# eigenkernel/eigenkernel

Measured on AMD Instinct MI355X. Metric: eigenpairs/s (full spectrum) + achieved fp64 TFLOP/s vs roofline, N=16384 GEP, higher is better.
Workload: dtype f64

## Files before the change

eigenkernel_amd/csrc/ek_api.hip:

```cpp
#include "ek_api_internal.h"

#include <cfloat>

namespace ek {
namespace api {

Context g_ctx;
std::mutex g_mu;

int ensure_init() {
  if (g_ctx.ready) return 0;
  int ndev = 0;
  EK_HIP_CHECK(hipGetDeviceCount(&ndev));
  if (ndev <= 0) {
    fprintf(stderr, "[ek_hip] no HIP device visible: this library has no CPU fallback\n");
    return -1000 - (int)hipErrorNoDevice;
  }
  EK_HIP_CHECK(hipSetDevice(g_ctx.device));
  EK_HIP_CHECK(hipStreamCreateWithFlags(&g_ctx.stream, hipStreamNonBlocking));
  {
    int lo = 0, hi = 0;
    (void)hipDeviceGetStreamPriorityRange(&lo, &hi);
    EK_HIP_CHECK(hipStreamCreateWithPriority(&g_ctx.stream2, hipStreamNonBlocking, hi));
  }
  EK_HIP_CHECK(hipMalloc((void **)&g_ctx.d_info, 64 * sizeof(int)));
  EK_HIP_CHECK(hipMalloc((void **)&g_ctx.d_status, 64));
  EK_HIP_CHECK(hipMalloc((void **)&g_ctx.d_stats, 64));
  EK_HIP_CHECK(hipMemset(g_ctx.d_stats, 0, 64));
  g_ctx.ready = true;
  return 0;
}

namespace { void *g_uimg = nullptr; size_t g_uimg_bytes = 0; }
int user_images(size_t bytes, void **p) {
  if (bytes > g_uimg_bytes) {
    if (g_uimg) EK_HIP_CHECK(hipFree(g_uimg));
    g_uimg = nullptr; g_uimg_bytes = 0;
    EK_HIP_CHECK(hipMalloc(&g_uimg, bytes));
// ... 853 lines not shown
```

eigenkernel_amd/csrc/ek_api_internal.h:

```cpp
#pragma once
#include "../../include/ek_hip.h"
#include "../../include/ek_hip_debug.h"
#include "ek_common.h"
#include "ek_switch.h"

#include <rccl/rccl.h>

#include <chrono>
#include <cstdlib>
#include <cstring>
#include <mutex>
#include <vector>

namespace ek {
namespace batched {
struct Desc {
  double *A, *B, *w, *Z;
  int n, lda, ldb, ldz, index, pad;
};
static_assert(sizeof(Desc) == 56, "the table's entry");
struct WDesc {
  double vl, vu;
  int il, iu, zcap, wcols;
  long long lu;
};
static_assert(sizeof(WDesc) == 40, "the window table's entry");
}

namespace api {

struct Context {
  bool ready = false;
  int device = 0;
  hipStream_t stream = nullptr;
  hipStream_t stream2 = nullptr;
  void *ws = nullptr;
  void *ws_alloc = nullptr;
  size_t ws_bytes = 0;
  int *d_info = nullptr;
  double *d_status = nullptr;
  double *d_stats = nullptr;
  double stats[8] = {0, 0, 0, 0, 0, 0, 0, 0};
};
extern Context g_ctx;
extern std::mutex g_mu;

int ensure_init();
int workspace(size_t bytes, void **p);

struct Arena {
// ... 52 lines not shown
int d2h_matrix(int m, int n, const double *d, int ldd, double *h, int ldh, hipStream_t s);
int fetch_info(int *info);
void poison_foreign_strips(hipStream_t s, int n, double *A, int lda, int P, int rank);
void count_mismatch(hipStream_t s, int m, int n, const double *X, int ldx, const double *Y, int ldy, int lower,
                    unsigned long long *count);

struct Comm {
  bool on = false;
  bool host = false;
  ncclComm_t comm = nullptr;
  int nranks = 0, rank = 0;
  int err = 0;
};
extern Comm g_comm;
constexpr int kPotrfRlMin = 1024;
extern int g_two_stage_min;
int two_stage_min();
int dist_min_ranks();
void comm_teardown();
SytrdExchange team_exchange(int nteam, int n = 0);
void team_sendrecv(hipStream_t s, int npeers, const int *peers, double *const *send, const size_t *send_counts,
                   double *const *recv, const size_t *recv_counts);
int comm_any(int local);
int comm_agree(int local_rc);
const char *comm_error_string();

void gather_band_strips(hipStream_t s, int n, int nmem, int rank0, double *const *ABs, const SytrdExchange &x);

inline int hip_rc(hipError_t e) { return e == hipSuccess ? 0 : -1000 - (int)e; }
#define EK_TRY(call) do { const int rc_ = (call); if (rc_) return rc_; } while (0)
// ... 57 lines not shown
```

eigenkernel_amd/csrc/ek_chol.hip:

```cpp
#include "ek_common.h"
#include "ek_block64.h"

#include <cstdlib>
#include <vector>

namespace ek {
namespace {

constexpr int NB = kDiagNB;
constexpr size_t kDiagLds = 2 * b64::IMG * sizeof(double);

__global__ __launch_bounds__(256) void potrf_diag_kernel(int nb, double *B, int ldb, double *inv, int *info,
                                                         int info_base) {
  using namespace b64;
  extern __shared__ double smem[];
  double *sP = smem, *sQ = smem + IMG;
  __shared__ double s_scr[kScratch];
  const int t = threadIdx.x, lane = t & 63, wave = t >> 6, l15 = lane & 15, l4 = lane >> 4;
  auto upper = [&](int gr, int gc) -> double {
    if (gc < nb) return B[(size_t)gc + (size_t)gr * ldb];
    return (gr == gc) ? 1.0 : 0.0;
  };
  auto fail_exit = [&](int j) {
    if (t == 0) atomicCAS(info, 0, info_base + j + 1);
// ... 198 lines not shown
  static bool attr_set = false;
  if (attr_set) return;
  (void)hipFuncSetAttribute((const void *)potrf_diag_kernel, hipFuncAttributeMaxDynamicSharedMemorySize, kDiagLds);
  (void)hipFuncSetAttribute((const void *)trtri_diag_kernel,
                            hipFuncAttributeMaxDynamicSharedMemorySize, (NB * NB + NB) * sizeof(double));
  attr_set = true;
}

void potrf_lower(hipStream_t s, int n, double *B, int ldb, double *invdiag, int *d_info,
                 double *work) {
  set_attrs();
  if (n <= 0) return;
  potrf_rec(s, n, B, ldb, 0, invdiag, d_info, work);
}

void trtri256_blocks(hipStream_t s, int n, const double *L, int ldl, const double *invdiag, double *inv256, double *scratch) {
  const int nb2 = n / (2 * NB);
  if (nb2 <= 0) return;
  GemmDesc g{};
  g.M = NB; g.N = NB; g.K = NB; g.transA = false; g.transB = false; g.alpha = 1.0; g.beta = 0.0; g.batch = nb2; g.lower_only = false;
  g.A = L + NB; g.lda = ldl; g.strideA = (long long)2 * NB * ((long long)ldl + 1);
  g.B = invdiag; g.ldb = NB; g.strideB = (long long)2 * NB * NB;
  g.C = scratch; g.ldc = NB; g.strideC = (long long)NB * NB;
  gemm(s, g);
  g.alpha = -1.0;
  g.A = invdiag + (size_t)NB * NB; g.lda = NB; g.strideA = (long long)2 * NB * NB;
  g.B = scratch; g.ldb = NB; g.strideB = (long long)NB * NB;
  g.C = inv256 + NB; g.ldc = 2 * NB; g.strideC = (long long)4 * NB * NB;
  gemm(s, g);
  hipLaunchKernelGGL(inv256_assemble_kernel, dim3(nb2), dim3(256), 0, s, invdiag, inv256);
}
void trsm_register_inv256(const double *invdiag, const double *inv256, int n) {
  g_inv256.base128 = inv256 ? invdiag : nullptr; g_inv256.inv256 = inv256; g_inv256.nblk256 = inv256 ? n / (2 * NB) : 0;
// ... 124 lines not shown
  const int before = g_sygst_direct;
  g_sygst_direct = order <= 0 ? kSygstDirect : (order < 2 * NB ? 2 * NB : order);
  return before;
}
void sygst_scratch_need(int n, size_t need[2]) {
  if (n <= sygst_direct()) return;
  const size_t n1 = (size_t)split_t(n), n2 = (size_t)n - n1;
  const size_t t1 = n1 * n1 + n1 * n2, t2 = (n1 > n2 ? n1 : n2) * (size_t)n;
  if (t1 > need[0]) need[0] = t1;
  if (t2 > need[1]) need[1] = t2;
  sygst_scratch_need((int)n1, need);
  sygst_scratch_need((int)n2, need);
}

static void sygst_rec(hipStream_t s, int n, double *A, int lda, const double *L, int ldl,
                      const double *invdiag, double *work, double *scratch) {
  if (n <= 0) return;
  if (n <= sygst_direct()) {
    symmetrize_lower(s, n, A, lda);
    trsm_lln(s, n, n, L, ldl, invdiag, A, lda, work);
    trsm_rlt_lower(s, n, L, ldl, invdiag, A, lda, work);
    return;
  }
  const int n1 = split_t(n), n2 = n - n1;
  double *A21 = A + n1, *A22 = A + (size_t)n1 + (size_t)n1 * lda;
  const double *L21 = L + n1, *L22 = L + (size_t)n1 + (size_t)n1 * ldl;
  const double *inv2 = invdiag + (size_t)(n1 / NB) * NB * NB;
  sygst_rec(s, n1, A, lda, L, ldl, invdiag, work, scratch);
  trsm_rlt(s, n2, n1, L, ldl, invdiag, A21, lda, work);
  double *C11 = scratch, *M = scratch + (size_t)n1 * n1;
  hipLaunchKernelGGL(full_from_lower_kernel, grid_mn(n1, n1), dim3(256), 0, s, n1, A, lda, C11, n1);
  gemm(s, false, false, n2, n1, n1, 1.0, L21, ldl, C11, n1, 0.0, M, n2);
  hipLaunchKernelGGL(axpy_matrix_kernel, grid_mn(n2, n1), dim3(256), 0, s, n2, n1, -0.5, M, n2, A21, lda);
  if (n2 <= n1) {
    double *P = C11;
    gemm(s, false, true, n2, n2, n1, 1.0, A21, lda, L21, ldl, 0.0, P, n2);
    hipLaunchKernelGGL(syr2k_fold_kernel, dim3(ceil_div(n2, 32), ceil_div(n2, 32)), dim3(256), 0, s, n2, P, n2, A22, lda);
  } else {
    gemm(s, false, true, n2, n2, n1, -1.0, A21, lda, L21, ldl, 1.0, A22, lda, true);
    gemm(s, false, true, n2, n2, n1, -1.0, L21, ldl, A21, lda, 1.0, A22, lda, true);
  }
  hipLaunchKernelGGL(axpy_matrix_kernel, grid_mn(n2, n1), dim3(256), 0, s, n2, n1, -0.5, M, n2, A21, lda);
  trsm_lln(s, n2, n1, L22, ldl, inv2, A21, lda, work);
  sygst_rec(s, n2, A22, lda, L22, ldl, inv2, work, scratch);
}

void sygst_lower(hipStream_t s, int n, double *A, int lda, const double *L, int ldl,
                 const double *invdiag, double *work, double *scratch) {
  if (n <= 0) return;
  sygst_rec(s, n, A, lda, L, ldl, invdiag, work, scratch);
}


__global__ __launch_bounds__(256) void trmm_diag_kernel(int n, int ldd, const double *__restrict__ L, int ldl,
                                                        double *__restrict__ diag) {
  const int b = blockIdx.x, off = b * ldd;
  const int nb = n - off < ldd ? n - off : ldd;
  double *D = diag + (size_t)b * ldd * ldd;
  const int per = ldd * ldd / gridDim.y;
  for (int idx = blockIdx.y * per + threadIdx.x; idx < (blockIdx.y + 1) * per; idx += 256) {
    const int i = idx % ldd, j = idx / ldd;
    D[idx] = (i >= j && i < nb) ? L[(size_t)(off + i) + (size_t)(off + j) * ldl] : 0.0;
  }
}
int trmm_block_ld(int n) { return n > kDiagNB ? 2 * NB : NB; }
// ... 288 lines not shown
      if (e0) { g_pprof.mark(s); g_pprof.kind.push_back(1); }
      if (has_next) issue_strip(s, k + 1, cur ^ 1);
      waited = true;
    }
  }
  for (int m = 0; m < nmem; ++m)
    hipLaunchKernelGGL(info_to_double_kernel, dim3(ceil_div(NRB, 256)), dim3(256), 0, s, NRB, infos[m], infod[m]);
  x.allreduce(s, nmem, infod, (size_t)NRB, x.user);
  for (int m = 0; m < nmem; ++m)
    hipLaunchKernelGGL(first_info_kernel, dim3(1), dim3(64), 0, s, NRB, infod[m], mem[m].d_info);
}

size_t potrf_rl_work_bytes(int n, int ld) { return PotrfDistLayout(n, ld, 1).total; }

void potrf_lower_rl(hipStream_t s, hipStream_t s2, int n, double *B, int ldb, double *invdiag, int *d_info,
                    void *work) {
  set_attrs();
  if (n <= 0) return;
  const PotrfDistLayout Ly(n, ldb, 1);
  const int NRB = Ly.NRB;
  char *w = (char *)work;
  double *ppan = (double *)(w + Ly.off_pbuf);
  int *infos = (int *)(w + Ly.off_infos);
  double *infod = (double *)(w + Ly.off_infod);
  long long *offs = (long long *)(w + Ly.off_offs);
  int *dims = (int *)(w + Ly.off_dims);
  static hipEvent_t evU[2], evP[2], evFork;
  static bool ev_ready = false;
  if (!ev_ready) {
    for (int i = 0; i < 2; ++i) {
      (void)hipEventCreateWithFlags(&evU[i], hipEventDisableTiming);
      (void)hipEventCreateWithFlags(&evP[i], hipEventDisableTiming);
    }
    (void)hipEventCreateWithFlags(&evFork, hipEventDisableTiming);
    ev_ready = true;
  }
  (void)hipMemsetAsync(infos, 0, (size_t)NRB * sizeof(int), s);
  hipLaunchKernelGGL(potrf_table_kernel, dim3(NRB), dim3(round_up(Ly.maxb, 64)), 0, s, n, ldb, 1, 0, NRB, Ly.maxb,
                     offs, dims);
  auto factor_panel = [&](hipStream_t st, int k) {
    const int off = k * NB, nbk = (n - off < NB) ? n - off : NB, mrows = n - off - nbk;
    double *Bd = B + (size_t)off + (size_t)off * ldb;
    double *inv = invdiag + (size_t)k * NB * NB;
    hipLaunchKernelGGL(potrf_diag_kernel, dim3(1), dim3(256), kDiagLds, st, nbk, Bd,
                       ldb, inv, infos + k, off);
    if (mrows > 0) {
      gemm(st, false, true, mrows, nbk, nbk, 1.0, Bd + nbk, ldb, inv, NB, 0.0, ppan, mrows);
      copy_matrix(st, mrows, nbk, ppan, mrows, Bd + nbk, ldb);
    }
// ... 5 lines not shown
    for (int k = k0; k < k1; ++k) {
      factor_panel(st, k);
      const int cnt = k1 - 1 - k;
      if (cnt > 0) {
        const int nbk = (n - k * NB < NB) ? n - k * NB : NB;
        GemmDesc g{};
        g.N = NB; g.K = nbk; g.transA = false; g.transB = true; g.alpha = -1.0; g.beta = 1.0;
        g.A = B; g.lda = ldb; g.B = B; g.ldb = ldb; g.C = B; g.ldc = ldb; g.lower_only = true;
        g.even_offs = true;
        g.M = n - (k + 1) * NB; g.batch = cnt;
        g.d_offs = offs + (size_t)k * Ly.maxb * 3; g.d_dims = dims + (size_t)k * Ly.maxb * 3;
        gemm(st, g);
      }
    }
  };
  (void)hipEventRecord(evFork, s);
  (void)hipStreamWaitEvent(s2, evFork, 0);
  factor_outer(s2, 0);
  (void)hipEventRecord(evP[0], s2);
  for (int o = 0; o + 1 < NOB; ++o) {
    const int c0 = o * ob * NB, c1 = (o + 1) * ob * NB, kw = c1 - c0;
    const int m2 = n - c1;
    const int wnext = (m2 < ob * NB) ? m2 : ob * NB;
    (void)hipStreamWaitEvent(s, evP[o & 1], 0);
    const double *P = B + (size_t)c1 + (size_t)c0 * ldb;
    double *C = B + (size_t)c1 + (size_t)c1 * ldb;
    gemm(s, false, true, m2, wnext, kw, -1.0, P, ldb, P, ldb, 1.0, C, ldb, true);
    (void)hipEventRecord(evU[(o + 1) & 1], s);
    if (m2 > wnext)
      gemm(s, false, true, m2 - wnext, m2 - wnext, kw, -1.0, P + wnext, ldb, P + wnext, ldb, 1.0,
           C + (size_t)wnext + (size_t)wnext * ldb, ldb, true);
    (void)hipStreamWaitEvent(s2, evU[(o + 1) & 1], 0);
    factor_outer(s2, o + 1);
    (void)hipEventRecord(evP[(o + 1) & 1], s2);
  }
  (void)hipStreamWaitEvent(s, evP[(NOB - 1) & 1], 0);
  hipLaunchKernelGGL(info_to_double_kernel, dim3(ceil_div(NRB, 256)), dim3(256), 0, s, NRB, infos, infod);
  hipLaunchKernelGGL(first_info_kernel, dim3(1), dim3(64), 0, s, NRB, infod, d_info);
}

size_t sygst_dist_scratch_doubles(int n, int ld, int nranks) {
  const int NRB = ceil_div(n > 0 ? n : 1, NB);
  return (size_t)ld * NB * ceil_div(NRB, nranks > 0 ? nranks : 1);
}

void sygst_lower_dist(hipStream_t s, int n, int nmem, const SygstMember *mem, const SytrdExchange &x) {
  if (n <= 0 || nmem <= 0 || nmem > kMaxTeam) return;
  const int P = x.nranks;
  const int NRB = ceil_div(n, NB);
  const int wblk = ceil_div(NRB, P) * NB;
  size_t offs[kMaxTeam], counts[kMaxTeam];
  for (int r = 0; r < P; ++r) {
    long long c0 = (long long)r * wblk, c1 = c0 + wblk;
// ... 34 lines not shown
```

eigenkernel_amd/csrc/ek_common.h:

```cpp
#pragma once
#include <hip/hip_runtime.h>
#include <cstddef>
#include <cstdint>
#include <cstdio>

#define EK_HIP_CHECK(expr)                                                              \
  do {                                                                                  \
    hipError_t _e = (expr);                                                             \
    if (_e != hipSuccess) {                                                             \
      fprintf(stderr, "[ek_hip] %s failed at %s:%d: %s\n", #expr, __FILE__, __LINE__,   \
              hipGetErrorString(_e));                                                   \
      return -1000 - (int)_e;                                                           \
    }                                                                                   \
  } while (0)

namespace ek {

constexpr int kWave = 64;

inline int ceil_div(int a, int b) { return (a + b - 1) / b; }
inline int round_up(int a, int b) { return ceil_div(a, b) * b; }

struct GemmDesc {
  int M, N, K;
// ... 59 lines not shown
constexpr int kDiagNB = 128;
void potrf_lower(hipStream_t s, int n, double *B, int ldb, double *invdiag, int *d_info,
                 double *work );
void trtri_diag_blocks(hipStream_t s, int n, const double *L, int ldl, double *invdiag);
void trsm_rlt(hipStream_t s, int m, int n, const double *L, int ldl, const double *invdiag,
              double *X, int ldx, double *work);
void trsm_lln(hipStream_t s, int n, int m, const double *L, int ldl, const double *invdiag,
              double *X, int ldx, double *work);
void trsm_llt(hipStream_t s, int n, int m, const double *L, int ldl, const double *invdiag,
              double *X, int ldx, double *work);
inline size_t sygst_scratch_doubles(int n) {
  const size_t h = (size_t)(n / 2 + 128);
  const size_t a = 2 * h * h, b = 2 * 128 * 128;
  return a > b ? a : b;
}
void trtri256_blocks(hipStream_t s, int n, const double *L, int ldl, const double *invdiag, double *inv256, double *scratch);
void trsm_register_inv256(const double *invdiag, const double *inv256, int n);
void sygst_lower(hipStream_t s, int n, double *A, int lda, const double *L, int ldl,
                 const double *invdiag, double *work, double *scratch);
int sygst_set_direct(int order);
void sygst_scratch_need(int n, size_t need[2]);
int trmm_block_ld(int n);
size_t trmm_diag_doubles(int n);
void trmm_diag_blocks(hipStream_t s, int n, const double *L, int ldl, double *diag);
void trmm_rln(hipStream_t s, int m, int n, const double *L, int ldl, const double *diag, int ldd,
              double *X, int ldx, double *work);
void trmm_llt(hipStream_t s, int n, int m, const double *L, int ldl, const double *diag, int ldd,
              double *X, int ldx, double *work);
void trmm_lln(hipStream_t s, int n, int m, const double *L, int ldl, const double *diag, int ldd,
              double *X, int ldx, double *work);
void sygst2_lower(hipStream_t s, int n, double *A, int lda, const double *L, int ldl, const double *diag,
                  double *work, double *scratch);
struct SygstMember {
  double *A; int lda; const double *L; int ldl; const double *invdiag;
  double *work;
  double *scratch;
  int rank;
};
size_t potrf_rl_work_bytes(int n, int ld);
void potrf_lower_rl(hipStream_t s, hipStream_t s2, int n, double *B, int ldb, double *invdiag, int *d_info,
                    void *work);
struct SytrdExchange;
struct PotrfMember { double *B; int ldb; double *invdiag; int *d_info; void *work; int rank; };
size_t potrf_dist_work_bytes(int n, int ld, int nranks);
void potrf_lower_dist(hipStream_t s, hipStream_t s2, int n, int nmem, const PotrfMember *mem, const SytrdExchange &x);
void potrf_dist_set_lookahead(int on);
void potrf_dist_profile(bool on);
void potrf_dist_profile_collect(double *seconds, int P);
size_t sygst_dist_scratch_doubles(int n, int ld, int nranks);
void sygst_lower_dist(hipStream_t s, int n, int nmem, const SygstMember *mem, const SytrdExchange &x);

struct SytrdWork;
size_t sytrd_work_bytes(int n);
void sytrd_lower(hipStream_t s, int n, double *A, int lda, double *d, double *e, double *tau,
                 double *V, int ldv, void *work);

// ... 105 lines not shown
```

eigenkernel_amd/csrc/ek_debug.hip:

```cpp
#include "ek_api_internal.h"

using namespace ek;
using namespace ek::api;

extern "C" {

int ek_hip_potrf_team(int n, double *B_loc, const int desc_B[9], int nteam, long long *mismatch) {
  if (n < 0) return -1;
  if (!B_loc && n > 0) return -2;
  int rc = check_desc(desc_B, 3, n, n); if (rc) return rc;
  if (nteam < 0 || nteam > kMaxTeam) return -4;
  rc = ensure_init(); if (rc) return rc;
  if (mismatch) *mismatch = 0;
  if (n == 0) return 0;
  std::lock_guard<std::mutex> lk(g_mu);
  if (nteam == 0 && !g_comm.on) return -4;
  hipStream_t s = g_ctx.stream;
  const int ld = pad_ld(n), nblk = ceil_div(n, kDiagNB);
  const int nmem = nteam > 0 ? nteam : 1, P = nteam > 0 ? nteam : g_comm.nranks;
  const size_t wb = potrf_dist_work_bytes(n, ld, P);
  const size_t per = al((size_t)ld * ld * 8) + al((size_t)nblk * kDiagNB * kDiagNB * 8) + al(wb) + 256;
  void *ws;
  rc = workspace(per * nmem + 256, &ws);
  if (rc) return rc;
// ... 206 lines not shown
  return sy2sb_on_host_arrays(n, A, lda, V, ldv, tau, 0, flag);
}

int ek_hip_debug_sy2sb_stage(int n, double *A, int lda, double *V, int ldv, double *tau, int poison, int *flag) {
  if (n < 1) return -1;
  if (!A) return -2;
  if (lda < n) return -3;
  if (!V) return -4;
  if (ldv < n) return -5;
  if (!tau) return -6;
  if (!flag) return -8;
  return sy2sb_on_host_arrays(n, A, lda, V, ldv, tau, poison, flag);
}

int ek_hip_debug_set_sy2sb_flow(int pair_min, int lookahead_min) { sy2sb_set_flow(pair_min, lookahead_min); return 0; }

__global__ void band_to_matrix_kernel(int n, const double *__restrict__ AB, double *__restrict__ A, int lda) {
  const int c = blockIdx.x;
  for (int d = threadIdx.x; d <= kBandW; d += blockDim.x)
    if (c + d < n) A[(size_t)(c + d) + (size_t)c * lda] = AB[(size_t)d + (size_t)c * kBandLd];
}

int ek_hip_debug_sy2sb_team(int n, double *A, int lda, double *V, int ldv, double *tau, int nteam, int *flag,
                            long long *mismatch) {
  if (n < 1 || !A || !V || !tau || lda < n || ldv < n) return -1;
  if (nteam < 0 || nteam > kMaxTeam) return -7;
  int rc = ensure_init(); if (rc) return rc;
  std::lock_guard<std::mutex> lk(g_mu);
  if (nteam == 0 && !g_comm.on) return -7;
  hipStream_t s = g_ctx.stream;
// ... 705 lines not shown
```

eigenkernel_amd/csrc/ek_solve.hip:

```cpp
#include "ek_api_internal.h"

namespace ek {
namespace api {

void gather_band_strips(hipStream_t s, int n, int nmem, int rank0, double *const *ABs, const SytrdExchange &x) {
  const int NRB = ceil_div(n, 128), P = x.nranks;
  if (P <= 1) return;
  for (int q = 0; q * P < NRB; ++q) {
    size_t offs[kMaxTeam], counts[kMaxTeam];
    for (int r = 0; r < P; ++r) {
      const int S = q * P + r;
      const int cols = (S < NRB) ? ((n - S * 128 < 128) ? n - S * 128 : 128) : 0;
      offs[r] = (S < NRB) ? (size_t)S * 128 * kBandLd : 0; counts[r] = (size_t)cols * kBandLd;
    }
    x.allgatherv(s, nmem, rank0, ABs, offs, counts, P, x.user);
  }
}

}
}

using namespace ek;
using namespace ek::api;

namespace {

struct StageTimer {
  hipEvent_t ev[EK_HIP_N_STAGES + 1];
  int made = 0;
  int init() {
    for (auto &e : ev) { EK_HIP_CHECK(hipEventCreate(&e)); ++made; }
    return 0;
// ... 20 lines not shown
  p.two_stage = ts_min > 0 && n >= ts_min && n >= 3;
  p.mat = al((size_t)p.ld * p.ld * 8);
  p.compact_dc = stedc_compact(n, nc_loc);
  p.zcols = p.compact_dc ? round_up(nc_loc > 0 ? nc_loc : 1, 128) : p.ld;
  p.zmat = al((size_t)p.ld * p.zcols * 8);
  p.wb_sytrd = (p.two_stage) ? 0 : (dist ? sytrd_dist_work_bytes(n, nranks_dist) : sytrd_work_bytes(n));
  p.wb_stedc = stedc_work_bytes(n, nc_loc);
  p.wb_ormtr = ormtr_work_bytes(n, nc_loc, n_vec);
  p.trsm_work = al((size_t)256 * p.ld * 8);
  p.inv256 = (problem == 1) ? al((size_t)(n / 256 > 0 ? n / 256 : 1) * 256 * 256 * 8) : 0;
  p.sygst_dbl = (problem == 1) ? sygst_scratch_doubles(n) : 0;
  if (problem == 1 && dist) {
    const size_t dd = sygst_dist_scratch_doubles(n, p.ld, nranks_dist);
    if (dd > p.sygst_dbl) p.sygst_dbl = dd;
  }
  p.potrf_rl = problem == 1 && n >= kPotrfRlMin;
  p.potrf_wb = (problem == 1 && dist) ? al(potrf_dist_work_bytes(n, p.ld, nranks_dist)) : 0;
  if (p.potrf_rl && al(potrf_rl_work_bytes(n, p.ld)) > p.potrf_wb) p.potrf_wb = al(potrf_rl_work_bytes(n, p.ld));
  p.wb_sy2sb = p.two_stage ? al(dist ? sy2sb_dist_work_bytes(n, nranks_dist) : sy2sb_work_bytes(n)) : 0;
  p.wb_sb2st = p.two_stage ? al(sb2st_work_bytes(n, false)) : 0;
  p.wb_rec = p.two_stage ? al(sb2st_record_bytes(n)) : 0;
  p.wb_q1prep = p.two_stage ? al(ormtr_prep_bytes(n)) : 0;
  p.x0 = p.mat;
  const size_t phase_a = al(p.sygst_dbl * 8) + p.potrf_wb + al(p.wb_sytrd) + 512;
  p.x1 = phase_a;
  if (values_only) {
    p.zcols = 0; p.zmat = 0; p.wb_stedc = 0; p.wb_ormtr = 0; p.wb_rec = 0; p.wb_q1prep = 0;
    if (al(stebz_work_bytes(n)) > p.x1) p.x1 = al(stebz_work_bytes(n));
    if (p.x1 < 4096) p.x1 = 4096;
  }
  if (al(p.wb_stedc) > p.x1) p.x1 = al(p.wb_stedc);
// ... 20 lines not shown
  int run();
  int rc = 0;
  hipStream_t s = g_ctx.stream;
  int nc_out = 0, nr_loc = 0, nc_loc = 0;
  bool dist = false, split_rows = false, values_only = false, value_window = false;
  PathPlan pl{};
  int ld = 0;
  bool two_stage = false, aliasA = false, aliasB = false, aliasZ = false;
  double *wB = nullptr, *wV = nullptr, *wZ = nullptr, *x0 = nullptr, *dInv = nullptr, *twork = nullptr, *dd = nullptr,
         *de = nullptr, *dt = nullptr, *dwv = nullptr, *dt1 = nullptr, *inv256 = nullptr;
  char *x1 = nullptr, *work_sy2sb = nullptr, *work_sb2st = nullptr, *q1prep = nullptr;
  double *wA = nullptr, *wV2 = nullptr;
  double *sscr = nullptr; char *pwork = nullptr; void *sytrd_work = nullptr;
  char *work = nullptr; double *q2rec = nullptr;
  Inv256Guard inv256_guard;
  StageTimer tm;
  bool timing = false;
  int evi = 0;
  void mark() { if (timing) (void)hipEventRecord(tm.ev[evi++], s); }
  double sigma = 1.0;
  bool band_input = false;
  bool two_stage_done = false, window_too_small = false;
  double rescued_panels = 0.0;
  int zslab = 0;
  int stage_in_A(), stage_in_B(), reduce(), tridiagonalise(), chase_with_repeat(), count_window(), values_tail(),
      divide_and_conquer(), stage_out(), finish(bool full), slab_width(int c0) const;
  void cholesky(), a_out(), back_transform(), recover(), z_out(int c0, int nc), exchange_rows();
};

Path::Path(const PathCall &call) : PathCall(call) {
// ... 34 lines not shown
  dd = a.get<double>(ld); de = a.get<double>(ld); dt = a.get<double>(ld); dwv = a.get<double>(ld);
  dt1 = a.get<double>(ld);
  work_sy2sb = two_stage ? a.get<char>(pl.wb_sy2sb) : nullptr;
  work_sb2st = two_stage ? a.get<char>(pl.wb_sb2st) : nullptr;
  q1prep = (two_stage && !values_only) ? a.get<char>(pl.wb_q1prep) : nullptr;
  inv256 = pl.inv256 ? (double *)a.get<char>(pl.inv256) : nullptr;
  wA = aliasA ? dA : x0;
  wV2 = x0;
  sscr = (problem == 1) ? (double *)x1 : nullptr;
  pwork = pl.potrf_wb ? x1 + al(pl.sygst_dbl * 8) : nullptr;
  work = x1;
  q2rec = (double *)x1;
  char *sytrd_arena = x1 + al(pl.sygst_dbl * 8) + pl.potrf_wb + 256;
  sytrd_work = two_stage ? nullptr : choose_sytrd_scratch(n, ld, x0, sytrd_arena, dd, pl.wb_sytrd);
  timing = stage_seconds && n_stages > 0;
}

int Path::run() {
  if (rc) return rc;
  if (timing) EK_TRY(tm.init());
  EK_HIP_CHECK(hipMemsetAsync(g_ctx.d_info, 0, 4 * sizeof(int), s));
  mark();
  EK_HIP_CHECK(hipMemsetAsync(wV, 0, (size_t)ld * ld * 8, s));
  EK_HIP_CHECK(hipMemsetAsync(dd, 0, 4 * al((size_t)ld * 8), s));
  if (!pipe) EK_TRY(stage_in_A());
  EK_TRY(stage_in_B());
  mark();
  cholesky();
  mark();
  if (pipe) {
    EK_TRY(stage_in_A());
    if (problem == 1) {
      if (!aliasB) copy_matrix(s, n, n, wB, ld, dB, ldb);
      pipe_out(pipe, s, 'B', dB, ldb, n, 0, n);
    }
  }
  EK_TRY(reduce());
  mark();
  EK_TRY(tridiagonalise());
  mark();
  EK_TRY(count_window());
  if (values_only || (win && (win->m == 0 || window_too_small))) return values_tail();
  EK_TRY(divide_and_conquer());
  mark();
  back_transform();
  mark();
  recover();
  mark();
  EK_TRY(stage_out());
  mark();
  return finish(true);
}
// ... 22 lines not shown
  for (int q = 0; q < 256; ++q) { if (part[q] > anrm) anrm = part[q]; if (!(part[256 + q] <= offband)) offband = part[256 + q]; }
  band_input = switch_int(kSwBandInput) != 0 && problem == 0 && !dist && offband == 0.0;
  if (!(anrm <= 1.7e308)) return -4;
  const double rmin = 1e-90, rmax = 1e90;
  if (anrm > 0.0 && anrm < rmin) sigma = rmin / anrm;
  else if (anrm > rmax) sigma = rmax / anrm;
  if (sigma != 1.0) scale_lower(s, n, sigma, wA, ld);
  return 0;
}

void Path::cholesky() {
  if (problem == 1) {
    if (dist && g_comm.nranks >= dist_min_ranks()) {
      const PotrfMember me{wB, ld, dInv, g_ctx.d_info, pwork, g_comm.rank};
      potrf_lower_dist(s, g_ctx.stream2, n, 1, &me, team_exchange(0));
    } else if (pl.potrf_rl) {
      potrf_lower_rl(s, g_ctx.stream2, n, wB, ld, dInv, g_ctx.d_info, pwork);
    } else {
      potrf_lower(s, n, wB, ld, dInv, g_ctx.d_info, twork);
    }
  }
  if (problem == 1 && n >= 256 && (itype == 1 || (itype == 2 && !values_only))) {
    trtri256_blocks(s, n, wB, ld, dInv, inv256, twork);
    trsm_register_inv256(dInv, inv256, n);
  }
}

int Path::reduce() {
  if (problem != 1) return 0;
  if (dist && g_comm.nranks >= dist_min_ranks()) {
    const SygstMember me{wA, ld, wB, ld, dInv, twork, sscr, g_comm.rank};
    sygst_lower_dist(s, n, 1, &me, team_exchange(0));
  } else if (itype == 1) {
    sygst_lower(s, n, wA, ld, wB, ld, dInv, twork, sscr);
  } else {
    trmm_diag_blocks(s, n, wB, ld, wV);
    sygst2_lower(s, n, wA, ld, wB, ld, wV, twork, sscr);
    EK_HIP_CHECK(hipMemsetAsync(wV, 0, trmm_diag_doubles(n) * 8, s));
  }
  return 0;
}

void Path::a_out() {
  if (!aliasA) copy_matrix(s, n, n, wA, ld, dA, lda);
  if (pipe) pipe_out(pipe, s, 'A', dA, lda, n, 0, n);
}

int Path::tridiagonalise() {
  if (dist && !two_stage) {
// ... 180 lines not shown
    const double *src = (i == cell->myrow) ? own : rp[q++];
    scatter_block_cyclic(s, nr_loc, nc_i, src, ldp, nb, 1, 0, R, i, dZ, ldz);
  }
}

int Path::finish(bool full) {
  EK_HIP_CHECK(hipGetLastError());
  int info[4] = {0, 0, 0, 0};
  EK_HIP_CHECK(hipMemcpyAsync(info, g_ctx.d_info, sizeof(info), hipMemcpyDeviceToHost, s));
  if (full) EK_HIP_CHECK(hipMemcpyAsync(g_ctx.stats, g_ctx.d_stats, sizeof(g_ctx.stats), hipMemcpyDeviceToHost, s));
  EK_HIP_CHECK(hipStreamSynchronize(s));
  if (!full) g_ctx.stats[0] = 0.0;
  g_ctx.stats[1] = two_stage_done ? 1.0 : 0.0;
  g_ctx.stats[2] = rescued_panels;
  g_ctx.stats[3] = (two_stage_done && band_input) ? 1.0 : 0.0;
  if (timing) {
    float ms[8];
    for (int i = 0; i < 8; ++i) (void)hipEventElapsedTime(&ms[i], tm.ev[i], tm.ev[i + 1]);
    double st[EK_HIP_N_STAGES] = {0};
    st[EK_STAGE_COPY] = (ms[0] + ms[7]) * 1e-3;
    st[EK_STAGE_POTRF] = ms[1] * 1e-3; st[EK_STAGE_SYGST] = ms[2] * 1e-3;
    st[EK_STAGE_SYTRD] = ms[3] * 1e-3; st[EK_STAGE_STEDC] = ms[4] * 1e-3;
    if (full) { st[EK_STAGE_ORMTR] = ms[5] * 1e-3; st[EK_STAGE_TRTRS] = ms[6] * 1e-3; }
    for (int i = 0; i < n_stages && i < EK_HIP_N_STAGES; ++i) stage_seconds[i] = st[i];
  }
  if (full) {
    int bad = two_stage_done && (info[2] & 0xff) != 0;
    if (dist) {
      bad = comm_any(bad);
      if (bad < 0) {
// ... 223 lines not shown
```

eigenkernel_amd/solver.py:

```python
import ctypes
import os
from dataclasses import dataclass, field

import numpy as np

from . import descriptor as _d

_HERE = os.path.dirname(os.path.abspath(__file__))
LIB_PATH = os.environ.get("EK_HIP_LIB") or os.path.join(_HERE, "csrc", "libek_hip.so")

N_STAGES = 8
SOLVERS = ("hip", "hip_select", "general_hip", "general_hip_select")
REPLACES = {"hip": "scalapack", "hip_select": "scalapack_select",
            "general_hip": "general_scalapack", "general_hip_select": "general_scalapack_select"}


class LibraryMissing(RuntimeError):
    pass


_lib = None
_dp = ctypes.POINTER(ctypes.c_double)
_ip = ctypes.POINTER(ctypes.c_int)
_llp = ctypes.POINTER(ctypes.c_longlong)
# ... 64 lines not shown
        "ek_hip_debug_sytrd_work_bytes": (ctypes.c_ulonglong, [c_int]),
        "ek_hip_debug_sytrd_split": (c_int, [vp, c_int]),
        "ek_hip_debug_gemm_at": (c_int, [c_int, c_int, c_int, c_int, c_int, vp, c_int, vp, c_int, c_dbl, vp, c_int,
                                         c_int, c_int, _dp]),
        "ek_hip_debug_sytrd_at": (c_int, [c_int, c_int, c_int, vp, vp, vp, _dp]),
        "ek_hip_debug_gemm_desc": (c_int, [c_int] * 5 + [c_dbl, c_dbl, vp, c_int, c_ll, vp, c_int, c_ll, vp, c_int, c_ll]
                                   + [c_int] * 5 + [_llp, _ip, _ip]),
        "ek_hip_debug_gemm_plan": (c_int, [c_int] * 5 + [c_dbl, c_dbl, vp, c_int, c_ll, vp, c_int, c_ll, vp, c_int, c_ll]
                                   + [c_int] * 5 + [_llp, _ip, _ip]),
        "ek_hip_debug_gemm_compact_map": (c_int, [c_int, c_int, c_ll, c_int, _ip, _ip, _ip]),
        "ek_hip_debug_reduce_team": (c_int, [c_int, c_int, c_int, _dp]),
        "ek_hip_profile_symv_get": (c_int, [_dp, ctypes.POINTER(ctypes.c_longlong), _dp]),
        "ek_hip_debug_sy2sb": (c_int, [c_int, _dp, c_int, _dp, c_int, _dp, _ip]),
        "ek_hip_debug_sy2sb_stage": (c_int, [c_int, _dp, c_int, _dp, c_int, _dp, c_int, _ip]),
        "ek_hip_debug_set_sy2sb_flow": (c_int, [c_int, c_int]),
        "ek_hip_debug_sb2st": (c_int, [c_int, _dp, c_int, _dp, _dp, _dp, c_int, c_int, _ip]),
        "ek_hip_debug_sb2st_stage": (c_int, [c_int, _dp, c_int, c_int, c_int, _dp, _dp, _dp, c_int, _dp, c_int, _dp, c_int,
                                             c_int, _ip, _ip]),
        "ek_hip_debug_two_stage_timing": (c_int, [c_int, c_int, c_int, _dp, _ip]),
        "ek_hip_debug_set_two_stage": (c_int, [c_int]),
        "ek_hip_profile_kernels": (c_int, [c_int]),
        "ek_hip_profile_kernels_get": (c_int, [_dp, _llp]),
        "ek_hip_debug_last_solve_stats": (c_int, [_dp, c_int]),
        "ek_hip_debug_sy2sb_team": (c_int, [c_int, _dp, c_int, _dp, c_int, _dp, c_int, _ip, _llp]),
        "ek_hip_debug_sy2sb_team_timing": (c_int, [c_int, c_int, c_int, _dp]),
        "ek_hip_debug_sy2sb_team_profile": (c_int, [c_int, c_int, c_int, c_int, _dp, _dp]),
        "ek_hip_debug_fail_next_chase": (c_int, [c_int]),
        "ek_hip_debug_stedc_team": (c_int, [c_int, c_int, c_int]),
        "ek_hip_debug_potrf_team_profile": (c_int, [c_int, c_int]),
        "ek_hip_debug_potrf_team_profile_get": (c_int, [c_int, _dp]),
# ... 159 lines not shown


EXPORTED_SYMBOLS = (
    "ek_hip_version", "ek_hip_init", "ek_hip_finalize", "ek_hip_stage_name", "ek_hip_solve",
    "ek_hip_solve_device", "ek_hip_solve_replicated", "ek_hip_solve_device_grid",
    "ek_hip_set_allgatherv", "ek_hip_gather_matrix", "ek_hip_potrf", "ek_hip_sygst", "ek_hip_sytrd", "ek_hip_stedc",
    "ek_hip_ormtr", "ek_hip_trtrs", "ek_hip_dgemm", "ek_hip_malloc", "ek_hip_free",
    "ek_hip_memcpy_h2d", "ek_hip_memcpy_d2h", "ek_hip_synchronize", "ek_hip_synth_matrix_device",
    "ek_hip_profile_symv", "ek_hip_profile_symv_get", "ek_hip_debug_sytrd",
    "ek_hip_residual_device", "ek_hip_orthogonality_device", "ek_hip_ipratios_device", "ek_hip_check",
    "ek_hip_sytrd_team", "ek_hip_comm_unique_id", "ek_hip_comm_init", "ek_hip_comm_size", "ek_hip_comm_rank",
    "ek_hip_comm_destroy", "ek_hip_comm_allreduce_device", "ek_hip_debug_sytrd_team", "ek_hip_sygst_team",
    "ek_hip_potrf_team", "ek_hip_debug_reduce_team", "ek_hip_comm_attach_host",
    "ek_hip_debug_set_sytrd_maxcols", "ek_hip_debug_sytrd_work_bytes", "ek_hip_debug_sytrd_at", "ek_hip_debug_sytrd_split", "ek_hip_debug_gemm_at",
    "ek_hip_debug_gemm_desc", "ek_hip_debug_gemm_plan", "ek_hip_debug_gemm_compact_map",
    "ek_hip_debug_sy2sb", "ek_hip_debug_sy2sb_stage", "ek_hip_debug_set_sy2sb_flow", "ek_hip_debug_sb2st", "ek_hip_debug_sb2st_stage", "ek_hip_debug_two_stage_timing", "ek_hip_debug_set_two_stage",
    "ek_hip_profile_kernels", "ek_hip_profile_kernels_get", "ek_hip_debug_last_solve_stats",
    "ek_hip_debug_sy2sb_team", "ek_hip_debug_sy2sb_team_timing", "ek_hip_debug_sy2sb_team_profile", "ek_hip_debug_workspace_bytes", "ek_hip_debug_fail_next_chase", "ek_hip_debug_last_pipe_stats",
    "ek_hip_debug_stedc_team", "ek_hip_debug_stedc_team_get", "ek_hip_debug_stedc",
    "ek_hip_debug_stedc_zcols", "ek_hip_debug_ormtr",
    "ek_hip_debug_potrf_team_profile", "ek_hip_debug_potrf_team_profile_get",
    "ek_hip_eigenvalues_device", "ek_hip_eigenvalues", "ek_hip_stebz",
    "ek_hip_debug_values_workspace_bytes", "ek_hip_debug_set_stebz",
    "ek_hip_eigenpairs_device", "ek_hip_eigenpairs", "ek_hip_stebz_range", "ek_hip_debug_window_workspace_bytes",
    "ek_hip_sygvx_device", "ek_hip_sygvx", "ek_hip_sygst_ibtype", "ek_hip_trmm", "ek_hip_debug_sygvx_workspace_bytes",
    "ek_hip_eigenpairs_batched_device", "ek_hip_eigenpairs_batched",
    "ek_hip_eigenpairs_vbatched_device", "ek_hip_eigenpairs_vbatched",
    "ek_hip_debug_vbatched_streams", "ek_hip_debug_vbatched_last",
    "ek_hip_check_batched_device", "ek_hip_check_batched", "ek_hip_check_vbatched_device", "ek_hip_check_vbatched",
    "ek_hip_sygv_batched_device", "ek_hip_sygv_batched", "ek_hip_sygv_vbatched_device", "ek_hip_sygv_vbatched",
    "ek_hip_check_sygv_batched_device", "ek_hip_check_sygv_batched", "ek_hip_check_sygv_vbatched_device",
# ... 1064 lines not shown
def sy2sb_stage(A, poison=False):
    lib = load_library()
    A = np.array(_farr(A), order="F", copy=True)
    n = A.shape[0]
    V = np.zeros((n, n), order="F"); tau = np.zeros(max(n, 1)); flag = ctypes.c_int(-1)
    rc = lib.ek_hip_debug_sy2sb_stage(n, _P(A), max(1, n), _P(V), max(1, n), _P(tau), 1 if poison else 0, ctypes.byref(flag))
    if rc:
        raise RuntimeError("ek_hip_debug_sy2sb_stage info=%d" % rc)
    return A, V, tau[:n], flag.value


def set_sy2sb_flow(pair_min=-1, lookahead_min=-1):
    rc = load_library().ek_hip_debug_set_sy2sb_flow(int(pair_min), int(lookahead_min))
    if rc:
        raise RuntimeError("ek_hip_debug_set_sy2sb_flow info=%d" % rc)


def sy2sb_team(A, nteam):
    lib = load_library()
    A = np.array(_farr(A), order="F", copy=True)
    n = A.shape[0]
    V = np.zeros((n, n), order="F"); tau = np.zeros(max(n, 1)); flag = ctypes.c_int(-1); mism = ctypes.c_longlong(-1)
    rc = lib.ek_hip_debug_sy2sb_team(n, _P(A), max(1, n), _P(V), max(1, n), _P(tau), int(nteam), ctypes.byref(flag),
                                     ctypes.byref(mism))
    if rc:
        raise RuntimeError("ek_hip_debug_sy2sb_team info=%d" % rc)
    return A, V, tau[:n], flag.value, mism.value


def sb2st(Bd, Z=None):
# ... 246 lines not shown
```

include/ek_hip_debug.h:

```cpp
#ifndef EK_HIP_DEBUG_H
#define EK_HIP_DEBUG_H

#ifdef __cplusplus
extern "C" {
#endif

int ek_hip_profile_symv(int enable);
int ek_hip_profile_symv_get(double *seconds, long long *launches, double *algorithmic_bytes);

int ek_hip_profile_kernels(int enable);
int ek_hip_profile_kernels_get(double *seconds , long long *launches );

int ek_hip_debug_sytrd(int n, int ld, int reps, double *seconds);
unsigned long long ek_hip_debug_sytrd_work_bytes(int n);
int ek_hip_debug_sytrd_at(int n, int max_cols, int reps, double *dA, void *work, double *vecs, double *seconds);
int ek_hip_debug_gemm_at(int transa, int transb, int m, int n, int k, const double *dA, int lda, const double *dB,
                         int ldb, double beta, double *dC, int ldc, int lower_only, int reps, double *seconds);
int ek_hip_debug_gemm_desc(int transa, int transb, int m, int n, int k, double alpha, double beta, const double *dA, int lda,
                           long long strideA, const double *dB, int ldb, long long strideB, double *dC, int ldc,
                           long long strideC, int batch, int lower_only, int staged_rank_k, int small_tiles, int even_offs,
                           const long long *offs, const int *dims, int *variant );
int ek_hip_debug_gemm_plan(int transa, int transb, int m, int n, int k, double alpha, double beta, const double *dA, int lda,
                           long long strideA, const double *dB, int ldb, long long strideB, double *dC, int ldc,
                           long long strideC, int batch, int lower_only, int staged_rank_k, int small_tiles, int even_offs,
// ... 29 lines not shown
                                                             int n_check, int index1, int index2, int n_ipr);
long long ek_hip_debug_sparse_csr(int n, long long nnz, const int *suf, const double *val, long long *rowptr, int *col,
                                  double *csr_val);
int ek_hip_debug_vbatched_streams(int streams);
int ek_hip_debug_vbatched_last(double *class_seconds, int *class_count);
int ek_hip_debug_xvbatched_last(double *class_seconds, int *class_count);
int ek_hip_debug_xbatched_chunk(int problems);
int ek_hip_debug_window_batched_chunk(int problems);
int ek_hip_debug_window_xbatched_chunk(int problems);
long long ek_hip_debug_window_xvbatched_budget(long long bytes);
int ek_hip_debug_check_xbatched_chunk(int problems);
int ek_hip_debug_check_xvbatched_last(double class_seconds[4], int class_count[4]);

int ek_hip_debug_stage_leaves256(int mode);
int ek_hip_debug_set_sygst_direct(int order);
unsigned long long ek_hip_debug_sygst_scratch(int n, unsigned long long *need );

int ek_hip_debug_fail_next_chase(int times);

int ek_hip_debug_stedc_team(int nranks, int levels, int profile);
int ek_hip_debug_stedc_team_get(double *seconds);

int ek_hip_debug_stedc(int n, const double *d, const double *e, int nsel, int first, int nb, int npcol, int mycol,
                       double *w, double *Z, int ldz, int *merges, int merge_cap, int *info);
int ek_hip_debug_stedc_zcols(int n, int nsel);

int ek_hip_debug_ormtr(int n, int ncols, const double *V, int ldv, const double *tau, double *Z, int ldz,
                       int ncols_global, int slab);

int ek_hip_debug_potrf_team_profile(int lookahead, int profile);
// ... 9 lines not shown
```

Measured before the change: 20500.

## Overlap trailing Cholesky factorization with the first sygst recursion half

Potrf is split at the sygst recursion split point. Trailing-block updates and the final info kernels after that point move to a third high-priority stream, and trtri for the leading diagonal blocks runs right away. Sygst's first-half work proceeds on the main stream and only joins the Cholesky tail, then inverts the remaining diagonal blocks, just before it needs L22. This hides part of the Cholesky critical path behind the GEP reduction, at the cost of more cross-stream events and SM contention between the two streams.

Result: no change. 20660, median of 6 (+0.8%).

```diff
diff --git a/eigenkernel_amd/csrc/ek_api.hip b/eigenkernel_amd/csrc/ek_api.hip
--- a/eigenkernel_amd/csrc/ek_api.hip
+++ b/eigenkernel_amd/csrc/ek_api.hip
@@ -22,6 +22,9 @@
     int lo = 0, hi = 0;
     (void)hipDeviceGetStreamPriorityRange(&lo, &hi);
     EK_HIP_CHECK(hipStreamCreateWithPriority(&g_ctx.stream2, hipStreamNonBlocking, hi));
+    EK_HIP_CHECK(hipStreamCreateWithPriority(&g_ctx.stream3, hipStreamNonBlocking, hi));
+    EK_HIP_CHECK(hipEventCreateWithFlags(&g_ctx.ev_chol_split, hipEventDisableTiming));
+    EK_HIP_CHECK(hipEventCreateWithFlags(&g_ctx.ev_chol_end, hipEventDisableTiming));
   }
   EK_HIP_CHECK(hipMalloc((void **)&g_ctx.d_info, 64 * sizeof(int)));
   EK_HIP_CHECK(hipMalloc((void **)&g_ctx.d_status, 64));
diff --git a/eigenkernel_amd/csrc/ek_api_internal.h b/eigenkernel_amd/csrc/ek_api_internal.h
--- a/eigenkernel_amd/csrc/ek_api_internal.h
+++ b/eigenkernel_amd/csrc/ek_api_internal.h
@@ -34,6 +34,8 @@
   int device = 0;
   hipStream_t stream = nullptr;
   hipStream_t stream2 = nullptr;
+  hipStream_t stream3 = nullptr;
+  hipEvent_t ev_chol_split = nullptr, ev_chol_end = nullptr;
   void *ws = nullptr;
   void *ws_alloc = nullptr;
   size_t ws_bytes = 0;
@@ -116,6 +118,8 @@
 };
 extern Comm g_comm;
 constexpr int kPotrfRlMin = 1024;
+extern int g_potrf_rl_min, g_chol_overlap_min;
+inline int potrf_rl_min() { return g_potrf_rl_min < 0 ? kPotrfRlMin : g_potrf_rl_min; }
 extern int g_two_stage_min;
 int two_stage_min();
 int dist_min_ranks();
diff --git a/eigenkernel_amd/csrc/ek_chol.hip b/eigenkernel_amd/csrc/ek_chol.hip
--- a/eigenkernel_amd/csrc/ek_chol.hip
+++ b/eigenkernel_amd/csrc/ek_chol.hip
@@ -236,9 +236,13 @@
   potrf_rec(s, n, B, ldb, 0, invdiag, d_info, work);
 }
 
-void trtri256_blocks(hipStream_t s, int n, const double *L, int ldl, const double *invdiag, double *inv256, double *scratch) {
-  const int nb2 = n / (2 * NB);
+void trtri256_blocks(hipStream_t s, int n, const double *L, int ldl, const double *invdiag, double *inv256, double *scratch,
+                     int c0, int c1) {
+  const int b0 = c0 / (2 * NB), nb2 = (c1 < 0 ? n : c1) / (2 * NB) - b0;
   if (nb2 <= 0) return;
+  L += (size_t)b0 * 2 * NB * ((size_t)ldl + 1);
+  invdiag += (size_t)b0 * 2 * NB * NB;
+  inv256 += (size_t)b0 * 4 * NB * NB;
   GemmDesc g{};
   g.M = NB; g.N = NB; g.K = NB; g.transA = false; g.transB = false; g.alpha = 1.0; g.beta = 0.0; g.batch = nb2; g.lower_only = false;
   g.A = L + NB; g.lda = ldl; g.strideA = (long long)2 * NB * ((long long)ldl + 1);
@@ -393,7 +397,7 @@
 }
 
 static void sygst_rec(hipStream_t s, int n, double *A, int lda, const double *L, int ldl,
-                      const double *invdiag, double *work, double *scratch) {
+                      const double *invdiag, double *work, double *scratch, const SygstJoin *join = nullptr) {
   if (n <= 0) return;
   if (n <= sygst_direct()) {
     symmetrize_lower(s, n, A, lda);
@@ -420,14 +424,20 @@
     gemm(s, false, true, n2, n2, n1, -1.0, L21, ldl, A21, lda, 1.0, A22, lda, true);
   }
   hipLaunchKernelGGL(axpy_matrix_kernel, grid_mn(n2, n1), dim3(256), 0, s, n2, n1, -0.5, M, n2, A21, lda);
+  if (join) join->fn(s, join->user);
   trsm_lln(s, n2, n1, L22, ldl, inv2, A21, lda, work);
   sygst_rec(s, n2, A22, lda, L22, ldl, inv2, work, scratch);
 }
 
+int sygst_split(int n) { return n > sygst_direct() ? split_t(n) : 0; }
 void sygst_lower(hipStream_t s, int n, double *A, int lda, const double *L, int ldl,
-                 const double *invdiag, double *work, double *scratch) {
-  if (n <= 0) return;
-  sygst_rec(s, n, A, lda, L, ldl, invdiag, work, scratch);
+                 const double *invdiag, double *work, double *scratch, const SygstJoin *join) {
+  if (n <= 0 || n <= sygst_direct()) {
+    if (join) join->fn(s, join->user);
+    if (n <= 0) return;
+    join = nullptr;
+  }
+  sygst_rec(s, n, A, lda, L, ldl, invdiag, work, scratch, join);
 }
 
 
@@ -746,7 +756,7 @@
 size_t potrf_rl_work_bytes(int n, int ld) { return PotrfDistLayout(n, ld, 1).total; }
 
 void potrf_lower_rl(hipStream_t s, hipStream_t s2, int n, double *B, int ldb, double *invdiag, int *d_info,
-                    void *work) {
+                    void *work, const PotrfSplit *split) {
   set_attrs();
   if (n <= 0) return;
   const PotrfDistLayout Ly(n, ldb, 1);
@@ -757,7 +767,7 @@
   double *infod = (double *)(w + Ly.off_infod);
   long long *offs = (long long *)(w + Ly.off_offs);
   int *dims = (int *)(w + Ly.off_dims);
-  static hipEvent_t evU[2], evP[2], evFork;
+  static hipEvent_t evU[2], evP[2], evFork, evTail;
   static bool ev_ready = false;
   if (!ev_ready) {
     for (int i = 0; i < 2; ++i) {
@@ -765,6 +775,7 @@
       (void)hipEventCreateWithFlags(&evP[i], hipEventDisableTiming);
     }
     (void)hipEventCreateWithFlags(&evFork, hipEventDisableTiming);
+    (void)hipEventCreateWithFlags(&evTail, hipEventDisableTiming);
     ev_ready = true;
   }
   (void)hipMemsetAsync(infos, 0, (size_t)NRB * sizeof(int), s);
@@ -800,29 +811,42 @@
       }
     }
   };
+  const int o_split = split ? (split->n1 - 1) / (ob * NB) : -1;
+  hipStream_t su = s;
+  auto split_behind = [&](int o) {
+    if (o != o_split) return;
+    (void)hipEventRecord(split->ev_split, s2);
+    (void)hipEventRecord(evTail, s);
+    (void)hipStreamWaitEvent(split->s3, evTail, 0);
+    (void)hipStreamWaitEvent(s, split->ev_split, 0);
+    su = split->s3;
+  };
   (void)hipEventRecord(evFork, s);
   (void)hipStreamWaitEvent(s2, evFork, 0);
   factor_outer(s2, 0);
   (void)hipEventRecord(evP[0], s2);
+  split_behind(0);
   for (int o = 0; o + 1 < NOB; ++o) {
     const int c0 = o * ob * NB, c1 = (o + 1) * ob * NB, kw = c1 - c0;
     const int m2 = n - c1;
     const int wnext = (m2 < ob * NB) ? m2 : ob * NB;
-    (void)hipStreamWaitEvent(s, evP[o & 1], 0);
+    (void)hipStreamWaitEvent(su, evP[o & 1], 0);
     const double *P = B + (size_t)c1 + (size_t)c0 * ldb;
     double *C = B + (size_t)c1 + (size_t)c1 * ldb;
-    gemm(s, false, true, m2, wnext, kw, -1.0, P, ldb, P, ldb, 1.0, C, ldb, true);
-    (void)hipEventRecord(evU[(o + 1) & 1], s);
+    gemm(su, false, true, m2, wnext, kw, -1.0, P, ldb, P, ldb, 1.0, C, ldb, true);
+    (void)hipEventRecord(evU[(o + 1) & 1], su);
     if (m2 > wnext)
-      gemm(s, false, true, m2 - wnext, m2 - wnext, kw, -1.0, P + wnext, ldb, P + wnext, ldb, 1.0,
+      gemm(su, false, true, m2 - wnext, m2 - wnext, kw, -1.0, P + wnext, ldb, P + wnext, ldb, 1.0,
            C + (size_t)wnext + (size_t)wnext * ldb, ldb, true);
     (void)hipStreamWaitEvent(s2, evU[(o + 1) & 1], 0);
     factor_outer(s2, o + 1);
     (void)hipEventRecord(evP[(o + 1) & 1], s2);
-  }
-  (void)hipStreamWaitEvent(s, evP[(NOB - 1) & 1], 0);
-  hipLaunchKernelGGL(info_to_double_kernel, dim3(ceil_div(NRB, 256)), dim3(256), 0, s, NRB, infos, infod);
-  hipLaunchKernelGGL(first_info_kernel, dim3(1), dim3(64), 0, s, NRB, infod, d_info);
+    split_behind(o + 1);
+  }
+  (void)hipStreamWaitEvent(su, evP[(NOB - 1) & 1], 0);
+  hipLaunchKernelGGL(info_to_double_kernel, dim3(ceil_div(NRB, 256)), dim3(256), 0, su, NRB, infos, infod);
+  hipLaunchKernelGGL(first_info_kernel, dim3(1), dim3(64), 0, su, NRB, infod, d_info);
+  if (split) (void)hipEventRecord(split->ev_end, su);
 }
 
 size_t sygst_dist_scratch_doubles(int n, int ld, int nranks) {
diff --git a/eigenkernel_amd/csrc/ek_common.h b/eigenkernel_amd/csrc/ek_common.h
--- a/eigenkernel_amd/csrc/ek_common.h
+++ b/eigenkernel_amd/csrc/ek_common.h
@@ -97,10 +97,13 @@
   const size_t a = 2 * h * h, b = 2 * 128 * 128;
   return a > b ? a : b;
 }
-void trtri256_blocks(hipStream_t s, int n, const double *L, int ldl, const double *invdiag, double *inv256, double *scratch);
+void trtri256_blocks(hipStream_t s, int n, const double *L, int ldl, const double *invdiag, double *inv256, double *scratch,
+                     int c0 = 0, int c1 = -1);
 void trsm_register_inv256(const double *invdiag, const double *inv256, int n);
+struct SygstJoin { void (*fn)(hipStream_t s, void *user); void *user; };
+int sygst_split(int n);
 void sygst_lower(hipStream_t s, int n, double *A, int lda, const double *L, int ldl,
-                 const double *invdiag, double *work, double *scratch);
+                 const double *invdiag, double *work, double *scratch, const SygstJoin *join = nullptr);
 int sygst_set_direct(int order);
 void sygst_scratch_need(int n, size_t need[2]);
 int trmm_block_ld(int n);
@@ -121,8 +124,9 @@
   int rank;
 };
 size_t potrf_rl_work_bytes(int n, int ld);
+struct PotrfSplit { int n1; hipStream_t s3; hipEvent_t ev_split, ev_end; };
 void potrf_lower_rl(hipStream_t s, hipStream_t s2, int n, double *B, int ldb, double *invdiag, int *d_info,
-                    void *work);
+                    void *work, const PotrfSplit *split = nullptr);
 struct SytrdExchange;
 struct PotrfMember { double *B; int ldb; double *invdiag; int *d_info; void *work; int rank; };
 size_t potrf_dist_work_bytes(int n, int ld, int nranks);
diff --git a/eigenkernel_amd/csrc/ek_debug.hip b/eigenkernel_amd/csrc/ek_debug.hip
--- a/eigenkernel_amd/csrc/ek_debug.hip
+++ b/eigenkernel_amd/csrc/ek_debug.hip
@@ -244,6 +244,13 @@
 }
 
 int ek_hip_debug_set_sy2sb_flow(int pair_min, int lookahead_min) { sy2sb_set_flow(pair_min, lookahead_min); return 0; }
+
+int ek_hip_debug_set_chol_overlap(int overlap_min, int potrf_rl_min) {
+  std::lock_guard<std::mutex> lk(g_mu);
+  g_chol_overlap_min = overlap_min < 0 ? -1 : overlap_min;
+  g_potrf_rl_min = potrf_rl_min < 0 ? -1 : potrf_rl_min;
+  return 0;
+}
 
 __global__ void band_to_matrix_kernel(int n, const double *__restrict__ AB, double *__restrict__ A, int lda) {
   const int c = blockIdx.x;
diff --git a/eigenkernel_amd/csrc/ek_solve.hip b/eigenkernel_amd/csrc/ek_solve.hip
--- a/eigenkernel_amd/csrc/ek_solve.hip
+++ b/eigenkernel_amd/csrc/ek_solve.hip
@@ -16,6 +16,8 @@
     x.allgatherv(s, nmem, rank0, ABs, offs, counts, P, x.user);
   }
 }
+
+int g_potrf_rl_min = -1, g_chol_overlap_min = -1;
 
 }
 }
@@ -66,7 +68,7 @@
     const size_t dd = sygst_dist_scratch_doubles(n, p.ld, nranks_dist);
     if (dd > p.sygst_dbl) p.sygst_dbl = dd;
   }
-  p.potrf_rl = problem == 1 && n >= kPotrfRlMin;
+  p.potrf_rl = problem == 1 && n >= potrf_rl_min();
   p.potrf_wb = (problem == 1 && dist) ? al(potrf_dist_work_bytes(n, p.ld, nranks_dist)) : 0;
   if (p.potrf_rl && al(potrf_rl_work_bytes(n, p.ld)) > p.potrf_wb) p.potrf_wb = al(potrf_rl_work_bytes(n, p.ld));
   p.wb_sy2sb = p.two_stage ? al(dist ? sy2sb_dist_work_bytes(n, nranks_dist) : sy2sb_work_bytes(n)) : 0;
@@ -117,6 +119,9 @@
   double *sscr = nullptr; char *pwork = nullptr; void *sytrd_work = nullptr;
   char *work = nullptr; double *q2rec = nullptr;
   Inv256Guard inv256_guard;
+  bool chol_overlap = false, chol_open = false, chol_forked = false;
+  void chol_join();
+  ~Path();
   StageTimer tm;
   bool timing = false;
   int evi = 0;
@@ -181,6 +186,20 @@
   char *sytrd_arena = x1 + al(pl.sygst_dbl * 8) + pl.potrf_wb + 256;
   sytrd_work = two_stage ? nullptr : choose_sytrd_scratch(n, ld, x0, sytrd_arena, dd, pl.wb_sytrd);
   timing = stage_seconds && n_stages > 0;
+  chol_overlap = pl.potrf_rl && !(dist && g_comm.nranks >= dist_min_ranks()) && itype == 1 && !pipe && sygst_split(n) > 0 &&
+                 n / 256 < 256 && (g_chol_overlap_min < 0 || (g_chol_overlap_min > 0 && n >= g_chol_overlap_min));
+}
+
+void Path::chol_join() {
+  if (!chol_open) return;
+  chol_open = false;
+  (void)hipStreamWaitEvent(s, g_ctx.ev_chol_end, 0);
+  trtri256_blocks(s, n, wB, ld, dInv, inv256, twork, sygst_split(n), -1);
+}
+Path::~Path() {
+  if (!chol_open) return;
+  (void)hipStreamWaitEvent(s, g_ctx.ev_chol_end, 0);
+  (void)hipStreamSynchronize(g_ctx.stream3);
 }
 
 int Path::run() {
@@ -202,7 +221,9 @@
       pipe_out(pipe, s, 'B', dB, ldb, n, 0, n);
     }
   }
-  EK_TRY(reduce());
+  const int reduce_rc = reduce();
+  chol_join();
+  EK_TRY(reduce_rc);
   mark();
   EK_TRY(tridiagonalise());
   mark();
@@ -255,6 +276,14 @@
     if (dist && g_comm.nranks >= dist_min_ranks()) {
       const PotrfMember me{wB, ld, dInv, g_ctx.d_info, pwork, g_comm.rank};
       potrf_lower_dist(s, g_ctx.stream2, n, 1, &me, team_exchange(0));
+    } else if (chol_overlap) {
+      const int n1 = sygst_split(n);
+      const PotrfSplit split{n1, g_ctx.stream3, g_ctx.ev_chol_split, g_ctx.ev_chol_end};
+      potrf_lower_rl(s, g_ctx.stream2, n, wB, ld, dInv, g_ctx.d_info, pwork, &split);
+      chol_open = chol_forked = true;
+      trtri256_blocks(s, n, wB, ld, dInv, inv256, twork, 0, n1);
+      trsm_register_inv256(dInv, inv256, n);
+      return;
     } else if (pl.potrf_rl) {
       potrf_lower_rl(s, g_ctx.stream2, n, wB, ld, dInv, g_ctx.d_info, pwork);
     } else {
@@ -273,7 +302,8 @@
     const SygstMember me{wA, ld, wB, ld, dInv, twork, sscr, g_comm.rank};
     sygst_lower_dist(s, n, 1, &me, team_exchange(0));
   } else if (itype == 1) {
-    sygst_lower(s, n, wA, ld, wB, ld, dInv, twork, sscr);
+    const SygstJoin join{[](hipStream_t, void *path) { ((Path *)path)->chol_join(); }, this};
+    sygst_lower(s, n, wA, ld, wB, ld, dInv, twork, sscr, chol_open ? &join : nullptr);
   } else {
     trmm_diag_blocks(s, n, wB, ld, wV);
     sygst2_lower(s, n, wA, ld, wB, ld, wV, twork, sscr);
@@ -484,6 +514,7 @@
   g_ctx.stats[1] = two_stage_done ? 1.0 : 0.0;
   g_ctx.stats[2] = rescued_panels;
   g_ctx.stats[3] = (two_stage_done && band_input) ? 1.0 : 0.0;
+  g_ctx.stats[4] = chol_forked ? 1.0 : 0.0;
   if (timing) {
     float ms[8];
     for (int i = 0; i < 8; ++i) (void)hipEventElapsedTime(&ms[i], tm.ev[i], tm.ev[i + 1]);
diff --git a/eigenkernel_amd/solver.py b/eigenkernel_amd/solver.py
--- a/eigenkernel_amd/solver.py
+++ b/eigenkernel_amd/solver.py
@@ -102,6 +102,7 @@
         "ek_hip_debug_sy2sb": (c_int, [c_int, _dp, c_int, _dp, c_int, _dp, _ip]),
         "ek_hip_debug_sy2sb_stage": (c_int, [c_int, _dp, c_int, _dp, c_int, _dp, c_int, _ip]),
         "ek_hip_debug_set_sy2sb_flow": (c_int, [c_int, c_int]),
+        "ek_hip_debug_set_chol_overlap": (c_int, [c_int, c_int]),
         "ek_hip_debug_sb2st": (c_int, [c_int, _dp, c_int, _dp, _dp, _dp, c_int, c_int, _ip]),
         "ek_hip_debug_sb2st_stage": (c_int, [c_int, _dp, c_int, c_int, c_int, _dp, _dp, _dp, c_int, _dp, c_int, _dp, c_int,
                                              c_int, _ip, _ip]),
@@ -291,7 +292,7 @@
     "ek_hip_potrf_team", "ek_hip_debug_reduce_team", "ek_hip_comm_attach_host",
     "ek_hip_debug_set_sytrd_maxcols", "ek_hip_debug_sytrd_work_bytes", "ek_hip_debug_sytrd_at", "ek_hip_debug_sytrd_split", "ek_hip_debug_gemm_at",
     "ek_hip_debug_gemm_desc", "ek_hip_debug_gemm_plan", "ek_hip_debug_gemm_compact_map",
-    "ek_hip_debug_sy2sb", "ek_hip_debug_sy2sb_stage", "ek_hip_debug_set_sy2sb_flow", "ek_hip_debug_sb2st", "ek_hip_debug_sb2st_stage", "ek_hip_debug_two_stage_timing", "ek_hip_debug_set_two_stage",
+    "ek_hip_debug_sy2sb", "ek_hip_debug_sy2sb_stage", "ek_hip_debug_set_sy2sb_flow", "ek_hip_debug_set_chol_overlap", "ek_hip_debug_sb2st", "ek_hip_debug_sb2st_stage", "ek_hip_debug_two_stage_timing", "ek_hip_debug_set_two_stage",
     "ek_hip_profile_kernels", "ek_hip_profile_kernels_get", "ek_hip_debug_last_solve_stats",
     "ek_hip_debug_sy2sb_team", "ek_hip_debug_sy2sb_team_timing", "ek_hip_debug_sy2sb_team_profile", "ek_hip_debug_workspace_bytes", "ek_hip_debug_fail_next_chase", "ek_hip_debug_last_pipe_stats",
     "ek_hip_debug_stedc_team", "ek_hip_debug_stedc_team_get", "ek_hip_debug_stedc",
@@ -1386,6 +1387,12 @@
     rc = load_library().ek_hip_debug_set_sy2sb_flow(int(pair_min), int(lookahead_min))
     if rc:
         raise RuntimeError("ek_hip_debug_set_sy2sb_flow info=%d" % rc)
+
+
+def set_chol_overlap(overlap_min=-1, potrf_rl_min=-1):
+    rc = load_library().ek_hip_debug_set_chol_overlap(int(overlap_min), int(potrf_rl_min))
+    if rc:
+        raise RuntimeError("ek_hip_debug_set_chol_overlap info=%d" % rc)
 
 
 def sy2sb_team(A, nteam):
diff --git a/include/ek_hip_debug.h b/include/ek_hip_debug.h
--- a/include/ek_hip_debug.h
+++ b/include/ek_hip_debug.h
@@ -67,6 +67,7 @@
 
 int ek_hip_debug_stage_leaves256(int mode);
 int ek_hip_debug_set_sygst_direct(int order);
+int ek_hip_debug_set_chol_overlap(int overlap_min, int potrf_rl_min);
 unsigned long long ek_hip_debug_sygst_scratch(int n, unsigned long long *need );
 
 int ek_hip_debug_fail_next_chase(int times);
```
